# aliftffd/ViT-vs-Raw-IQ

Measured on AMD Instinct MI355X. Metric: IQ frames/sec training (fwd+loss+bwd+clip+AdamW), higher is better.
Workload: dtype bf16; 1 GPU; ViT-Tiny/16 224x224 C=1 19cls (BASELINE configs[1]); config_id=B, per_gpu_batch=256, global_batch=256, parallelism=dp1, hipgraph=True

## Files before the change

include/iqvit.h:

```cpp
#ifndef IQVIT_H
#define IQVIT_H
#include <stddef.h>
#include <stdint.h>

#ifdef __cplusplus
extern "C" {
#endif

typedef void* iq_stream_t;

enum { IQ_STATUS_OK = 0, IQ_STATUS_ARG = 1, IQ_STATUS_UNSUPPORTED = 2, IQ_STATUS_LAUNCH = 3 };

typedef struct iq_dropout {
  uint64_t seed;
  uint32_t step;
  uint32_t site;
  float p;
  const uint32_t* step_dev;
} iq_dropout_t;
#define IQ_SITE_IMPAIR 0xFFFFFFFFu
#define IQ_SITE_SYNTH 0xFFFFFFFEu

int iq_ln_supported(int D);
int iq_ln_fwd(const void* z, const float* gamma, const float* beta, void* x, float* mean, float* rstd, int M, int D,
              float eps, iq_stream_t stream);
size_t iq_ln_bwd_ws_bytes(int D);
int iq_ln_bwd(const void* dx, const void* z, const float* mean, const float* rstd, const float* gamma, void* dz,
              void* dy, const iq_dropout_t* drop, float* dgamma, float* dbeta, float* ws, int accumulate, int M,
              int D, iq_stream_t stream);
int iq_ln_bwd_partial_rows(int M, int D);

typedef struct iq_epilogue {
  const float* bias;
  int relu;
  const float* pe;
  int tok, seq, cls_off;
  iq_dropout_t drop;
  const void* gate;
  int ldg;
  float gate_scale;
  const void* residual;
  int ldr;
} iq_epilogue_t;
int iq_gemm_bf16_nt(const void* A, int lda, const void* B, int ldb, void* C, int ldc, int M, int N, int K,
                    const iq_epilogue_t* epi, iq_stream_t stream);
// ... 48 lines not shown
  const float* partials;
  int rows;
  int64_t row_stride;
  float* out;
  int64_t n;
} iq_reduce_seg_t;
size_t iq_wgrad_grouped_ws_bytes(const iq_wgrad_problem_t* probs, int nprob, int M, int max_workgroups);
int iq_gemm_bf16_wgrad_grouped(const iq_wgrad_problem_t* probs, int nprob, int M, float* ws, size_t ws_bytes,
                               int accumulate, int max_workgroups, const iq_reduce_seg_t* extra, int nextra,
                               iq_stream_t stream);

int iq_attn_supported(int S, int dh);
int iq_attn_fwd(const void* qkv, void* out, float* lse, int B, int S, int H, int dh, iq_stream_t stream);
int iq_attn_bwd(const void* qkv, const void* out, const void* dout, const float* lse, void* dqkv, int B, int S, int H,
                int dh, iq_stream_t stream);
int iq_attn_fwd_masked(const void* qkv, void* out, float* lse, const uint8_t* mask, long mask_hstride, int B, int S,
                       int H, int dh, iq_stream_t stream);
int iq_attn_bwd_masked(const void* qkv, const void* out, const void* dout, const float* lse, void* dqkv,
                       const uint8_t* mask, long mask_hstride, int B, int S, int H, int dh, iq_stream_t stream);
int iq_attn_probs(const void* qkv, const float* lse, float* out, long out_bstride, int B, int S, int H, int dh,
                  int rows, int heads, iq_stream_t stream);
int iq_attn_grad_probs(const void* qkv, const float* lse, const void* dout, float* out, long out_bstride, int B, int S,
                       int H, int dh, int rows, int heads, int positive, iq_stream_t stream);
int iq_attn_relevance_step(const void* qkv, const float* lse, const void* dout, const float* r_in, float* r_out, int B,
                           int S, int H, int dh, iq_stream_t stream);

int iq_frames_preprocess(const float* raw, float* out, int n_frames, int len, int take, const float* stats,
                         iq_stream_t stream);
typedef struct iq_impair {
  float phase_lo, phase_hi;
// ... 103 lines not shown
```

vit-vs-raw-iq_amd/_native.py:

```python
from __future__ import annotations

import ctypes as C
import os

_HERE = os.path.dirname(os.path.abspath(__file__))
LIB_PATH = os.environ.get("IQ_LIBIQVIT") or os.path.join(_HERE, "libiqvit.so")

BWD_PARAM_GRADS = 1

STATUS = {0: "ok", 1: "invalid argument", 2: "unsupported shape/configuration", 3: "HIP launch error"}


class IqError(RuntimeError):
    pass


class Dropout(C.Structure):
    _fields_ = [("seed", C.c_uint64), ("step", C.c_uint32), ("site", C.c_uint32), ("p", C.c_float),
                ("step_dev", C.c_void_p)]


class Impair(C.Structure):
    _fields_ = [("phase_lo", C.c_float), ("phase_hi", C.c_float), ("cfo_lo", C.c_float), ("cfo_hi", C.c_float),
                ("rot90", C.c_int), ("conj", C.c_int), ("shift_max", C.c_int), ("gain_db_lo", C.c_float),
# ... 31 lines not shown
    _fields_ = [("kind", C.c_int), ("in_channels", C.c_int), ("img_h", C.c_int), ("img_w", C.c_int),
                ("patch", C.c_int), ("seq_length", C.c_int), ("conv_k", C.c_int), ("use_cls", C.c_int),
                ("num_classes", C.c_int), ("d_model", C.c_int), ("n_head", C.c_int), ("n_layers", C.c_int),
                ("ffn_hidden", C.c_int), ("drop_prob", C.c_float)]


_P, _I, _Z, _F = C.c_void_p, C.c_int, C.c_size_t, C.c_float
_U64, _U32 = C.c_uint64, C.c_uint32

SIGNATURES = {
    "iq_ln_supported": (_I, [_I]),
    "iq_ln_fwd": (_I, [_P, _P, _P, _P, _P, _P, _I, _I, _F, _P]),
    "iq_ln_bwd_ws_bytes": (_Z, [_I]),
    "iq_ln_bwd_partial_rows": (_I, [_I, _I]),
    "iq_ln_bwd": (_I, [_P, _P, _P, _P, _P, _P, _P, C.POINTER(Dropout), _P, _P, _P, _I, _I, _I, _P]),
    "iq_gemm_bf16_nt": (_I, [_P, _I, _P, _I, _P, _I, _I, _I, _I, C.POINTER(Epilogue), _P]),
    "iq_gemm_ln_supported": (_I, [_I, _I]),
    "iq_gemm_bf16_ln": (_I, [_P, _I, _P, _I, _P, _P, _I, C.POINTER(Dropout), _P, _P, _F, _P, _P, _P, _P, _I, _I, _I, _P]),
    "iq_gemm_lnbwd_supported": (_I, [_I, _I]),
    "iq_gemm_lnbwd_partial_rows": (_I, [_I]),
    "iq_gemm_bf16_lnbwd": (_I, [_P, _I, _P, _I, _P, _I, _P, _P, _P, _P, C.POINTER(Dropout), _P, _P, _P, _I, _I, _I, _P]),
    "iq_ffn_chain_supported": (_I, [_I, _I, _I]),
    "iq_ffn_chain_bwd_partial_rows": (_I, [_I]),
    "iq_ffn_chain_bwd": (_I, [_P, _P, _P, _F, _P, _P, _P, _P, _P, _P, _P, C.POINTER(Dropout), _P, _P, _P, _P, _P, _I, _I, _I, _I, _P]),
    "iq_qkv_dgrad_ffn_chain_bwd": (_I, [_P, _P, _P, _P, _P, _P, _P, C.POINTER(Dropout), _P, _P, _P,
                                        _P, _P, _F, _P, _P, _P, _P, _P, _P, _P, C.POINTER(Dropout), _P, _P, _P, _P, _P, _I, _I, _I, _I, _P]),
    "iq_ffn_chain_gate_bytes": (_Z, [_I, _I]),
    "iq_ffn_chain_fwd": (_I, [_P, _P, _P, C.POINTER(Dropout), _P, _P, _P, C.POINTER(Dropout), _P, _P, _F, _P, _P, _P, _P, _P, _I, _I,
                              _I, _I, _P]),
    "iq_attn_out_ffn_chain_fwd": (_I, [_P, _P, _P, C.POINTER(Dropout), _P, _P, _P, _P, _P, _P, _P,
                                       _P, _P, C.POINTER(Dropout), _P, _P, _P, C.POINTER(Dropout), _P, _P, _F, _P, _P, _P, _P, _P,
                                       _P, _P, _P, _I, _I, _I, _I, _P]),
    "iq_wgrad_ws_bytes": (_Z, [_I, _I, _I]),
    "iq_gemm_bf16_wgrad": (_I, [_P, _I, _P, _I, _P, _P, _I, _I, _I, _P, _Z, _I, _P]),
    "iq_wgrad_grouped_ws_bytes": (_Z, [_P, _I, _I, _I]),
    "iq_gemm_bf16_wgrad_grouped": (_I, [_P, _I, _I, _P, _Z, _I, _I, _P, _I, _P]),
    "iq_attn_supported": (_I, [_I, _I]),
    "iq_attn_fwd": (_I, [_P, _P, _P, _I, _I, _I, _I, _P]),
    "iq_attn_bwd": (_I, [_P, _P, _P, _P, _P, _I, _I, _I, _I, _P]),
    "iq_attn_fwd_masked": (_I, [_P, _P, _P, _P, C.c_long, _I, _I, _I, _I, _P]),
    "iq_attn_bwd_masked": (_I, [_P, _P, _P, _P, _P, _P, C.c_long, _I, _I, _I, _I, _P]),
    "iq_attn_probs": (_I, [_P, _P, _P, C.c_long, _I, _I, _I, _I, _I, _I, _P]),
    "iq_attn_grad_probs": (_I, [_P, _P, _P, _P, C.c_long, _I, _I, _I, _I, _I, _I, _I, _P]),
    "iq_attn_relevance_step": (_I, [_P, _P, _P, _P, _P, _I, _I, _I, _I, _P]),
    "iq_frames_preprocess": (_I, [_P, _P, _I, _I, _I, C.POINTER(C.c_float), _P]),
    "iq_frames_impair": (_I, [_P, _P, _P, _I, _I, _I, C.POINTER(C.c_float), C.POINTER(Impair), _P]),
    "iq_frames_synth": (_I, [_P, _P, _P, _P, _P, _I, _I, C.POINTER(Synth), _P]),
    "iq_patchify": (_I, [_P, _P, _I, _I, _I, _I, _I, _I, _I, _P]),
    "iq_cls_rows": (_I, [_P, _P, _P, _I, _I, _I, C.POINTER(Dropout), _P]),
    "iq_embed_bwd_gather": (_I, [_P, _P, _P, _I, _I, _I, _I, _I, C.POINTER(Dropout), _I, _P]),
    "iq_embed_dgrad": (_I, [_P, _P, _I, _P, _I, _I, _I, _I, _I, _I, _I, _P]),
    "iq_linf_step": (_I, [_P, _P, _P, _F, _F, _F, _F, _Z, _P]),
    "iq_head_fwd": (_I, [_P, _P, _P, _P, _P, _P, _P, _P, _I, _I, _I, _I, _I, _P]),
    "iq_ce_fwd_bwd": (_I, [_P, _P, _I, _I, _F, _F, _P, _P, _P, _P]),
# ... 70 lines not shown
```

vit-vs-raw-iq_amd/csrc/attention.hip:

```cpp

#include "common.h"
#include "iqvit.h"
#include "prof.h"

namespace {

constexpr int ATT_THREADS = 512;
constexpr int ATT_WAVES = ATT_THREADS / 64;
constexpr float LOG2E = 1.4426950408889634f;
constexpr float LN2 = 0.6931471805599453f;
constexpr float NEG_BIG = -1.0e30f;

__device__ __forceinline__ float fast_exp2(float x) { return __builtin_amdgcn_exp2f(x); }

template <int DH> struct AttCfg {
  static constexpr int LD = (DH == 16) ? 16 : DH + 16;
  static constexpr int KS = (DH + 31) / 32;
  static constexpr int DT = DH / 16;
  static constexpr int CPR = DH / 8;
};

typedef __attribute__((address_space(3))) s16x4 lds_s16x4;

__device__ __forceinline__ bf16x8 tr_frag(const bf16* tile, int ld, int r0, int c0, int lane) {
// ... 467 lines not shown
      for (int i = 0; i < NIMG; ++i) v[i][j] = *reinterpret_cast<const bf16x8*>(base[i] + (long)r * ldg[i] + c * 8);
    }
#pragma unroll
    for (int j = 0; j < UN; ++j) {
      const int id = b0 + j * NT + tid;
      const int r = id >> 3, c = id & 7;
      if (id < total) {
        const bool live = r < S;
#pragma unroll
        for (int i = 0; i < NIMG; ++i) *reinterpret_cast<bf16x8*>(img[i] + once_off(r, c * 8)) = live ? v[i][j] : bf16x8{};
      }
    }
  }
}

template <int NT>
__global__ __launch_bounds__(NT, 4) void attn_bwd_once_kernel(const bf16* __restrict__ qkv, const bf16* __restrict__ out,
                                                              const bf16* __restrict__ dout, const float* __restrict__ lse,
                                                              bf16* __restrict__ dqkv, int S, int H, int spad, float scale) {
  constexpr int DH = 64, KS = 2, DT = 4, NW = NT / 64;
  extern __shared__ __attribute__((aligned(16))) unsigned char smem[];
  bf16* I0 = reinterpret_cast<bf16*>(smem);
  bf16* I1 = I0 + spad * ONCE_LD;
  float* lse_s = reinterpret_cast<float*>(I1 + spad * ONCE_LD);
  float* del_s = lse_s + spad;
  bf16* dSi = reinterpret_cast<bf16*>(del_s + spad);
  const int tid = threadIdx.x, lane = tid & 63, wave = tid >> 6, g = lane >> 4, c16 = lane & 15;
  const int b = blockIdx.x / H, h = blockIdx.x % H;
  const int D = H * DH;
  const long ldg = 3L * D;
  const bf16* qb = qkv + (long)b * S * ldg + h * DH;
  const bf16* kb_ = qb + D;
  const bf16* vb_ = qb + 2 * D;
  const bf16* ob = out + (long)b * S * D + h * DH;
  const bf16* dob = dout + (long)b * S * D + h * DH;
  bf16* dqb = dqkv + (long)b * S * ldg + h * DH;
  const float scale_log2 = scale * LOG2E;
  const int nunit = (S + 15) / 16;
  const int ldS = nunit * 16 + 8;

  {
    bf16* const img[2] = {I0, I1};
    const bf16* const src[2] = {qb, dob};
    const long lds_[2] = {ldg, (long)D};
    once_stage<NT, 2048 / NT, 2>(img, src, lds_, spad, S, tid);
  }
  __syncthreads();
  for (int q = tid; q < spad; q += NT) {
    float dl = 0.f, ls = 0.f;
    if (q < S) {
#pragma unroll
      for (int c = 0; c < 8; ++c) {
        const bf16x8 a = *reinterpret_cast<const bf16x8*>(I1 + once_off(q, c * 8));
        const bf16x8 o8 = *reinterpret_cast<const bf16x8*>(ob + (long)q * D + c * 8);
#pragma unroll
        for (int e = 0; e < 8; ++e) dl += (float)a[e] * (float)o8[e];
      }
      ls = lse[((long)b * H + h) * S + q] * LOG2E;
    }
    del_s[q] = dl;
    lse_s[q] = ls;
  }
  __syncthreads();

  for (int unit = wave; unit < nunit; unit += NW) {
    bf16x8 kf[KS], vf[KS];
#pragma unroll
    for (int s = 0; s < KS; ++s) {
      kf[s] = row_frag_gmem<DH>(kb_, ldg, unit * 16 + c16, S, s, lane);
      vf[s] = row_frag_gmem<DH>(vb_, ldg, unit * 16 + c16, S, s, lane);
    }
    f32x4 dv[DT], dk[DT];
#pragma unroll
    for (int dt = 0; dt < DT; ++dt) { dv[dt] = f32x4{0.f, 0.f, 0.f, 0.f}; dk[dt] = f32x4{0.f, 0.f, 0.f, 0.f}; }
    const int key = unit * 16 + c16;
    const bool unit_partial = unit * 16 + 16 > S;
    for (int ql = 0; ql < spad; ql += 32) {
      const bool u1 = ql + 16 < S;
      f32x4 p[2], ds[2];
#pragma unroll
      for (int u = 0; u < 2; ++u) {
        if (u == 1 && !u1) { p[1] = f32x4{0.f, 0.f, 0.f, 0.f}; ds[1] = f32x4{0.f, 0.f, 0.f, 0.f}; continue; }
        f32x4 sa = {0.f, 0.f, 0.f, 0.f}, dp = {0.f, 0.f, 0.f, 0.f};
#pragma unroll
        for (int s = 0; s < KS; ++s) {
          const bf16x8 qa = once_row_frag(I0, ql + u * 16 + c16, s, lane);
          const bf16x8 da = once_row_frag(I1, ql + u * 16 + c16, s, lane);
          sa = __builtin_amdgcn_mfma_f32_16x16x32_bf16(qa, kf[s], sa, 0, 0, 0);
          dp = __builtin_amdgcn_mfma_f32_16x16x32_bf16(da, vf[s], dp, 0, 0, 0);
        }
        const f32x4 lq4 = *reinterpret_cast<const f32x4*>(lse_s + ql + u * 16 + 4 * g);
        const f32x4 dl4 = *reinterpret_cast<const f32x4*>(del_s + ql + u * 16 + 4 * g);
// ... 31 lines not shown
        *reinterpret_cast<bf16x4*>(dqb + (long)key * ldg + 2 * D + dt * 16 + 4 * g) = wv;
      }
    }
  }

  __syncthreads();
  {
    bf16* const img[1] = {I0};
    const bf16* const src[1] = {kb_};
    const long lds_[1] = {ldg};
    once_stage<NT, 2048 / NT, 1>(img, src, lds_, spad, S, tid);
  }
  __syncthreads();
  for (int half = wave; half < nunit; half += NW) {
    const int q = half * 16 + c16;
    const bf16* drow = dSi + q * ldS + 4 * g;
    f32x4 dq[DT];
#pragma unroll
    for (int dt = 0; dt < DT; ++dt) dq[dt] = f32x4{0.f, 0.f, 0.f, 0.f};
    for (int kl = 0; kl < spad; kl += 32) {
      const bool k1 = kl + 16 < S;
      const bf16x4 lo = *reinterpret_cast<const bf16x4*>(drow + kl);
      bf16x4 hi = {};
      if (k1) hi = *reinterpret_cast<const bf16x4*>(drow + kl + 16);
      const bf16x8 dsB = {lo[0], lo[1], lo[2], lo[3], hi[0], hi[1], hi[2], hi[3]};
#pragma unroll
      for (int dt = 0; dt < DT; ++dt) {
        const bf16x8 kT = once_tr_frag(I0, kl, dt, lane);
        dq[dt] = __builtin_amdgcn_mfma_f32_16x16x32_bf16(kT, dsB, dq[dt], 0, 0, 0);
      }
    }
    if (q < S) {
#pragma unroll
      for (int dt = 0; dt < DT; ++dt) {
        bf16x4 w;
#pragma unroll
        for (int r = 0; r < 4; ++r) w[r] = (bf16)dq[dt][r];
        *reinterpret_cast<bf16x4*>(dqb + (long)q * ldg + dt * 16 + 4 * g) = w;
      }
    }
  }
}

template <int DH>
__device__ __forceinline__ bf16x8 row_frag_img(const bf16* tile, int ld, int row, int s, int lane) {
  const int d0 = s * 32 + 8 * (lane >> 4);
  bf16x8 v = {};
  if (DH >= 32 || d0 < DH) v = *reinterpret_cast<const bf16x8*>(tile + row * ld + d0);
  return v;
}

template <int UN>
__device__ __forceinline__ void stage_block(bf16* img, int ld, const bf16* src, int cols, int S, int spad, int tid, int nthr) {
  const int cpr = cols >> 3, total = spad * cpr, live = S * cpr;
  for (int base = 0; base < total; base += UN * nthr) {
    bf16x8 v[UN];
// ... 410 lines not shown
               long mask_hstride, int B, int S, int H, hipStream_t st) {
  const int spad = (S + 31) / 32 * 32;
  const int chunk = bwd_chunk_rows<DH>(S);
  if (S > ATT_MAX_S || chunk < 32) return IQ_ERR_UNSUPPORTED;
  const size_t lds = bwd_lds_bytes<DH>(S);
  if (lds > 48 * 1024)
    (void)hipFuncSetAttribute((const void*)attn_bwd_kernel<DH, MASKED>, hipFuncAttributeMaxDynamicSharedMemorySize, (int)lds);
  attn_bwd_kernel<DH, MASKED><<<B * H, ATT_THREADS, lds, st>>>((const bf16*)qkv, (const bf16*)out, (const bf16*)dout, lse,
                                                               (bf16*)dqkv, mask, mask_hstride, S, H, spad, chunk,
                                                               1.0f / sqrtf((float)DH), -10000.0f * sqrtf((float)DH));
  return iq_launch_status();
}

constexpr int ONCE_THREADS = 1024;
inline bool use_once(int S, int dh, bool masked) { return !masked && dh == 64 && (S + 31) / 32 * 32 <= ONCE_MAX_SPAD; }
template <int NT>
int launch_bwd_once(const void* qkv, const void* out, const void* dout, const float* lse, void* dqkv, int B, int S, int H,
                    hipStream_t st) {
  const int spad = (S + 31) / 32 * 32, nunit = (S + 15) / 16;
  const size_t lds = (size_t)2 * spad * ONCE_LD * 2 + (size_t)2 * spad * sizeof(float) + (size_t)spad * (nunit * 16 + 8) * 2;
  auto k = attn_bwd_once_kernel<NT>;
  if (lds > 48 * 1024) (void)hipFuncSetAttribute((const void*)k, hipFuncAttributeMaxDynamicSharedMemorySize, (int)lds);
  k<<<B * H, NT, lds, st>>>((const bf16*)qkv, (const bf16*)out, (const bf16*)dout, lse, (bf16*)dqkv, S, H, spad,
                            1.0f / sqrtf(64.0f));
  return iq_launch_status();
}

template <bool MASKED>
int dispatch_fwd(const void* qkv, void* out, float* lse, const uint8_t* mask, long hs, int B, int S, int H, int dh,
                 hipStream_t st) {
  switch (dh) {
    case 16: return launch_fwd<16, MASKED>(qkv, out, lse, mask, hs, B, S, H, st);
    case 32: return launch_fwd<32, MASKED>(qkv, out, lse, mask, hs, B, S, H, st);
    case 64: return launch_fwd<64, MASKED>(qkv, out, lse, mask, hs, B, S, H, st);
    default: return IQ_ERR_UNSUPPORTED;
  }
}
template <bool MASKED>
int dispatch_bwd(const void* qkv, const void* out, const void* dout, const float* lse, void* dqkv, const uint8_t* mask,
                 long hs, int B, int S, int H, int dh, hipStream_t st) {
  switch (dh) {
    case 16: return launch_bwd<16, MASKED>(qkv, out, dout, lse, dqkv, mask, hs, B, S, H, st);
    case 32: return launch_bwd<32, MASKED>(qkv, out, dout, lse, dqkv, mask, hs, B, S, H, st);
    case 64: return launch_bwd<64, MASKED>(qkv, out, dout, lse, dqkv, mask, hs, B, S, H, st);
    default: return IQ_ERR_UNSUPPORTED;
  }
}

}

extern "C" int iq_attn_supported(int S, int dh) {
  if (S <= 0 || S > ATT_MAX_S) return 0;
  return (dh == 16 || dh == 32 || dh == 64) ? 1 : 0;
}

extern "C" int iq_attn_fwd_masked(const void* qkv, void* out, float* lse, const uint8_t* mask, long mask_hstride, int B,
                                  int S, int H, int dh, iq_stream_t stream) {
  if (B <= 0) return IQ_OK;
  if (!qkv || !out || !lse || S <= 0 || H <= 0) return IQ_ERR_ARG;
  if (mask_hstride != 0 && mask_hstride != (long)S * S) return IQ_ERR_ARG;
  hipStream_t st = (hipStream_t)stream;
// ... 37 lines not shown
  if (frame) {
    switch (dh) {
      case 16: return launch_frame_bwd<16>(qkv, out, dout, lse, dqkv, B, S, H, st);
      case 32: return launch_frame_bwd<32>(qkv, out, dout, lse, dqkv, B, S, H, st);
      default: return launch_frame_bwd<64>(qkv, out, dout, lse, dqkv, B, S, H, st);
    }
  }
  if (once) return launch_bwd_once<ONCE_THREADS>(qkv, out, dout, lse, dqkv, B, S, H, st);
  return mask ? dispatch_bwd<true>(qkv, out, dout, lse, dqkv, mask, mask_hstride, B, S, H, dh, st)
              : dispatch_bwd<false>(qkv, out, dout, lse, dqkv, nullptr, 0, B, S, H, dh, st);
}
extern "C" int iq_attn_bwd(const void* qkv, const void* out, const void* dout, const float* lse, void* dqkv, int B,
                           int S, int H, int dh, iq_stream_t stream) {
  return iq_attn_bwd_masked(qkv, out, dout, lse, dqkv, nullptr, 0, B, S, H, dh, stream);
}
```

vit-vs-raw-iq_amd/csrc/layernorm.hip:

```cpp
#include "common.h"
#include "iqvit.h"
#include "prof.h"

namespace {

template <int LPR>
__device__ __forceinline__ float group_sum(float v) {
#pragma unroll
  for (int o = LPR / 2; o > 0; o >>= 1) v += __shfl_xor(v, o, 64);
  return v;
}

constexpr int LN_THREADS = 256;

template <int LPR, int NV, bool MASK = false>
__global__ __launch_bounds__(LN_THREADS) void ln_fwd_kernel(const bf16* __restrict__ Z, const float* __restrict__ gamma,
                                                            const float* __restrict__ beta, bf16* __restrict__ X,
                                                            float* __restrict__ mean_out, float* __restrict__ rstd_out,
                                                            int M, int D, float eps) {
  constexpr int RPW = 64 / LPR;
  constexpr int RPB = RPW * (LN_THREADS / 64);
  const int lane = threadIdx.x & 63, wave = threadIdx.x >> 6;
  const int j = lane % LPR, rsub = lane / LPR;
  float g[NV][8], b[NV][8];
// ... 32 lines not shown
        float y[8];
#pragma unroll
        for (int e = 0; e < 8; ++e) y[e] = g[v][e] * ((x[v][e] - mean) * rstd) + b[v][e];
        if (!MASK || (v * LPR + j) * 8 < D) *reinterpret_cast<bf16x8*>(X + row * D + (v * LPR + j) * 8) = pack8(y);
      }
      if (j == 0) { mean_out[row] = mean; rstd_out[row] = rstd; }
    }
  }
}

template <int LPR, int NV, bool DROP, bool MASK = false>
__global__ __launch_bounds__(LN_THREADS) void ln_bwd_kernel(const bf16* __restrict__ dX, const bf16* __restrict__ Z,
                                                            const float* __restrict__ mean_in, const float* __restrict__ rstd_in,
                                                            const float* __restrict__ gamma, bf16* __restrict__ dZ,
                                                            bf16* __restrict__ dY, IqRng rng, uint32_t thresh, float dscale,
                                                            float* __restrict__ partial, int M, int D) {
  constexpr int RPW = 64 / LPR;
  constexpr int RPB = RPW * (LN_THREADS / 64);
  extern __shared__ __attribute__((aligned(16))) float red[];
  const int lane = threadIdx.x & 63, wave = threadIdx.x >> 6;
  const int j = lane % LPR, rsub = lane / LPR;
  float g[NV][8], ag[NV][8], ab[NV][8];
#pragma unroll
  for (int v = 0; v < NV; ++v) {
    const int c = (v * LPR + j) * 8;
#pragma unroll
    for (int e = 0; e < 8; ++e) { g[v][e] = (!MASK || c < D) ? gamma[c + e] : 0.f; ag[v][e] = 0.f; ab[v][e] = 0.f; }
  }
  const float invD = 1.0f / (float)D;
  if (DROP) rng = rng_resolve(rng);
  for (long row0 = (long)blockIdx.x * RPB; row0 < M; row0 += (long)gridDim.x * RPB) {
    const long row = row0 + wave * RPW + rsub;
    const bool ok = row < M;
    float xh[NV][8], dy[NV][8];
    float mean = 0.f, rstd = 0.f;
    if (ok) { mean = mean_in[row]; rstd = rstd_in[row]; }
    float s1 = 0.f, s2 = 0.f;
#pragma unroll
    for (int v = 0; v < NV; ++v) {
      bf16x8 tz = {}, td = {};
      const bool cv = !MASK || (v * LPR + j) * 8 < D;
      if (ok && cv) {
        tz = *reinterpret_cast<const bf16x8*>(Z + row * D + (v * LPR + j) * 8);
        td = *reinterpret_cast<const bf16x8*>(dX + row * D + (v * LPR + j) * 8);
      }
      unpack8(tz, xh[v]);
      unpack8(td, dy[v]);
#pragma unroll
      for (int e = 0; e < 8; ++e) {
        xh[v][e] = cv ? (xh[v][e] - mean) * rstd : 0.f;
        ag[v][e] += dy[v][e] * xh[v][e];
        ab[v][e] += dy[v][e];
        dy[v][e] *= g[v][e];
        s1 += dy[v][e];
        s2 += dy[v][e] * xh[v][e];
      }
    }
    const float c1 = group_sum<LPR>(s1) * invD;
    const float c2 = group_sum<LPR>(s2) * invD;
    if (ok) {
#pragma unroll
      for (int v = 0; v < NV; ++v) {
        float o[8];
#pragma unroll
        for (int e = 0; e < 8; ++e) o[e] = rstd * (dy[v][e] - c1 - xh[v][e] * c2);
        const long off = row * D + (v * LPR + j) * 8;
        if (MASK && (v * LPR + j) * 8 >= D) continue;
        *reinterpret_cast<bf16x8*>(dZ + off) = pack8(o);
        if (DROP) {
          const uint32_t keep = dropout_keep8(rng, (uint64_t)off >> 3, thresh);
#pragma unroll
          for (int e = 0; e < 8; ++e) o[e] = ((keep >> e) & 1u) ? o[e] * dscale : 0.f;
          *reinterpret_cast<bf16x8*>(dY + off) = pack8(o);
        }
      }
    }
  }
  const int rslot = wave * RPW + rsub;
#pragma unroll
  for (int v = 0; v < NV; ++v) {
    const int c = (v * LPR + j) * 8;
// ... 110 lines not shown

extern "C" size_t iq_ln_bwd_ws_bytes(int D) { return (size_t)LN_MAX_BLOCKS * 2 * D * sizeof(float); }

extern "C" int iq_ln_bwd_partial_rows(int M, int D) {
  LnShape s;
  if (M <= 0 || !ln_shape(D, &s)) return 0;
  int rows = 0;
  bool ok = ln_dispatch(s, [&](auto lpr, auto nv) {
    constexpr int LPR = decltype(lpr)::value;
    rows = ln_grid(M, (64 / LPR) * 4);
  });
  if (!ok) rows = ln_grid(M, 4);
  return rows;
}

extern "C" int iq_ln_bwd(const void* dx, const void* z, const float* mean, const float* rstd, const float* gamma,
                         void* dz, void* dy, const iq_dropout_t* drop, float* dgamma, float* dbeta, float* ws,
                         int accumulate, int M, int D, iq_stream_t stream) {
  LnShape s;
  if (M <= 0) return IQ_OK;
  if (!dx || !z || !mean || !rstd || !gamma || !dz || !ws) return IQ_ERR_ARG;
  if ((dgamma == nullptr) != (dbeta == nullptr)) return IQ_ERR_ARG;
  const bool reduce_now = dgamma != nullptr;
  if (!ln_shape(D, &s)) return IQ_ERR_UNSUPPORTED;
  int dropping; IqRng rng; uint32_t thresh; float dscale;
  (void)dropout_unpack(drop, &dropping, &rng, &thresh, &dscale);
  if (dropping && !dy) return IQ_ERR_ARG;
  hipStream_t st = (hipStream_t)stream;
  IQ_PROF(IQ_FAM_LN_BWD, st);
  IQ_PROF_K(2.0 * (double)M * D * (3 + (dropping ? 1 : 0)) + 8.0 * M, 0.0, "ln_bwd_kernel(D=%d)", D);
  int rc = IQ_OK;
  bool ok = ln_dispatch(s, [&](auto lpr, auto nv) {
    constexpr int LPR = decltype(lpr)::value, NV = decltype(nv)::value;
    constexpr int RPB = (64 / LPR) * 4;
    const int nblk = ln_grid(M, RPB);
    const size_t lds = (size_t)RPB * 2 * D * sizeof(float);
    if (lds > 160 * 1024) { rc = IQ_ERR_UNSUPPORTED; return; }
    if (dropping) {
      auto k = ln_bwd_kernel<LPR, NV, true>;
      if (lds > 48 * 1024) (void)hipFuncSetAttribute((const void*)k, hipFuncAttributeMaxDynamicSharedMemorySize, (int)lds);
      k<<<nblk, LN_THREADS, lds, st>>>((const bf16*)dx, (const bf16*)z, mean, rstd, gamma, (bf16*)dz, (bf16*)dy, rng,
                                       thresh, dscale, ws, M, D);
    } else {
      auto k = ln_bwd_kernel<LPR, NV, false>;
      if (lds > 48 * 1024) (void)hipFuncSetAttribute((const void*)k, hipFuncAttributeMaxDynamicSharedMemorySize, (int)lds);
      k<<<nblk, LN_THREADS, lds, st>>>((const bf16*)dx, (const bf16*)z, mean, rstd, gamma, (bf16*)dz, (bf16*)dy, rng,
                                       thresh, dscale, ws, M, D);
    }
    if (reduce_now) ln_bwd_reduce_kernel<<<(2 * D + 31) / 32, 1024, 0, st>>>(ws, nblk, D, dgamma, dbeta, accumulate);
  });
  if (!ok) ok = ln_dispatch_masked(D, [&](auto nv) {
    constexpr int NV = decltype(nv)::value;
    constexpr int RPB = 4;
    const int nblk = ln_grid(M, RPB);
    const size_t lds = (size_t)RPB * 2 * D * sizeof(float);
    if (dropping)
      ln_bwd_kernel<64, NV, true, true><<<nblk, LN_THREADS, lds, st>>>((const bf16*)dx, (const bf16*)z, mean, rstd, gamma,
                                                                      (bf16*)dz, (bf16*)dy, rng, thresh, dscale, ws, M, D);
    else
      ln_bwd_kernel<64, NV, false, true><<<nblk, LN_THREADS, lds, st>>>((const bf16*)dx, (const bf16*)z, mean, rstd, gamma,
                                                                       (bf16*)dz, (bf16*)dy, rng, thresh, dscale, ws, M, D);
    if (reduce_now) ln_bwd_reduce_kernel<<<(2 * D + 31) / 32, 1024, 0, st>>>(ws, nblk, D, dgamma, dbeta, accumulate);
  });
  if (!ok) return IQ_ERR_UNSUPPORTED;
  return rc != IQ_OK ? rc : iq_launch_status();
}
```

vit-vs-raw-iq_amd/csrc/model.hip:

```cpp
#include <hip/hip_runtime.h>
#include <stdio.h>
#include <string.h>

#include <string>
#include <vector>

#include "attn_maps.h"
#include "common.h"
#include "iqvit.h"
#include "prof.h"

int head_bwd_dx_launch(const float* dlogits, const float* featn, const float* hstat, const float* ln_g, const float* W, void* dx,
                       int B, int S, int D, int K, int pool, hipStream_t st);
int embed_bwd_gather_launch(const void* dx0, void* demb, int B, int S, int tok, int D, int has_cls, const iq_dropout_t* drop,
                            hipStream_t st);

namespace {

struct Entry {
  std::string name;
  size_t off;
  int ndim;
  int dims[4];
};
// ... 110 lines not shown
  std::vector<LayerOff> L;
  size_t hln_g, hln_b, head_w, head_b, head_begin;
  size_t sh_flat, sh_embw, sh_table, shadow_bytes;
  std::vector<TransDesc> ttab;
  int ttiles = 0;
  const void* table_uploaded_to = nullptr;
  float* params = nullptr;
  float* grads = nullptr;
  const float* pe = nullptr;
  unsigned char* shadow = nullptr;
  std::string err;
  uint32_t* step_ctr = nullptr;
  uint64_t last_seed = 0;
  bool last_tr = false;
  bool last_train_fwd = false;
  const void* fwd_ws = nullptr;
  int fwd_batch = 0;

  iq_dropout_t bwd_site(uint32_t id, const uint32_t* step_dev, bool tr) const {
    iq_dropout_t d;
    d.seed = last_seed; d.step = 0; d.site = id; d.p = tr ? c.drop_prob : 0.f; d.step_dev = step_dev;
    return d;
  }

  size_t add(const std::string& name, std::vector<int> dims, size_t& cur, bool aligned = true) {
    if (aligned) cur = align_up(cur, 64);
    Entry e;
    e.name = name; e.off = cur; e.ndim = (int)dims.size();
    size_t n = 1;
    for (int i = 0; i < 4; ++i) { e.dims[i] = i < e.ndim ? dims[i] : 1; n *= (size_t)e.dims[i]; }
// ... 446 lines not shown
  const WsPlan w = plan_ws(m, batch);
  if (ws_bytes < w.total) return fail(m, IQ_ERR_ARG, "backward: workspace too small");
  hipStream_t st = (hipStream_t)stream;
  unsigned char* ws = (unsigned char*)workspace;
  const int D = c.d_model, F = c.ffn_hidden, S = m->S, H = c.n_head, B = batch, K = c.num_classes;
  const int M = B * S, MT = B * m->tok;
  const bool tr = m->last_tr;
  const uint32_t* step_dev = m->step_ctr ? m->step_ctr : (const uint32_t*)(ws + w.step_ctr);
  const float* P = m->params;
  float* G = m->grads;
  float* wws = (float*)(ws + w.wgrad_ws);
  const float dscale = tr ? dropout_scale(c.drop_prob) : 1.f;

  if (stage_hi == Lr + 1) {
    if (!dlogits && !denc) return fail(m, IQ_ERR_ARG, "backward: dlogits or denc required at the head stage");
    if (dlogits && !pgrads) {
      IQ_TRY(head_bwd_dx_launch(dlogits, (const float*)(ws + w.head_feat), (const float*)(ws + w.head_stat),
                                m->head_ln ? P + m->hln_g : nullptr, P + m->head_w, ws + w.gA, B, S, D, K, m->pool, st), "head bwd (dx)");
    } else if (dlogits) {
      IQ_TRY(iq_head_bwd(dlogits, (const float*)(ws + w.head_feat), (const float*)(ws + w.head_stat),
                         m->head_ln ? P + m->hln_g : nullptr, m->head_ln ? P + m->hln_b : nullptr, P + m->head_w,
                         G + m->head_w, G + m->head_b, m->head_ln ? G + m->hln_g : nullptr,
                         m->head_ln ? G + m->hln_b : nullptr, ws + w.gA, B, S, D, K, m->pool, accumulate, stream), "head bwd");
    } else if (!accumulate && pgrads) {
      (void)hipMemsetAsync(G + m->head_begin, 0, (m->nparam - m->head_begin) * sizeof(float), st);
    }
    if (denc) f32_into_bf16_kernel<<<blocks_for((size_t)M * D / 8), 256, 0, st>>>(denc, (bf16*)(ws + w.gA), (size_t)M * D / 8, dlogits ? 1 : 0);
  }
  const bool fuse1 = iq_gemm_lnbwd_supported(D, F) != 0, fuse2 = iq_gemm_lnbwd_supported(D, 3 * D) != 0;
  const Route route = layer_route(M, S, D, F);
  const bool chain = fuse1 && m->last_train_fwd && route.chain;
  bool deferred = false;
  for (int sidx = (stage_hi > Lr ? Lr : stage_hi); sidx >= 1 && sidx >= stage_lo; --sidx) {
    const int l = sidx - 1;
    const LayerOff& o = m->L[l];
    const WsPlan::L& a = w.layers[l];
    const unsigned char* xin = l == 0 ? ws + w.x0 : ws + w.layers[l - 1].x2;
    unsigned char *gZ = ws + w.gZ, *gY = ws + w.gY, *gZ1 = ws + w.gZ1, *gY1 = ws + w.gY1;
    unsigned char *gH = ws + w.gH, *gQKV = ws + w.gQKV;
    iq_epilogue_t e;
    float* lp2 = (float*)(ws + w.ln_part[0]);
    float* lp1 = (float*)(ws + w.ln_part[1]);
    const bool norm2_here = l == Lr - 1 || !fuse2;
    if (norm2_here) {
      const iq_dropout_t dr2 = m->bwd_site(3 + 3 * l, step_dev, tr);
      IQ_TRY(iq_ln_bwd(ws + w.gA, ws + a.z2, (const float*)(ws + a.mean2), (const float*)(ws + a.rstd2), P + o.g2,
                       gZ, gY, &dr2, nullptr, nullptr, lp2, accumulate, M, D, stream), "norm2 bwd");
    }
    const unsigned char* dO2 = tr ? gY : gZ;
    const unsigned char* dAo = tr ? gY1 : gZ1;
    const iq_wgrad_problem_t wg[4] = {
        {dO2, D, ws + a.hid, F, G + o.w2, G + o.b2, D, F},
        {gH, F, ws + a.x1, D, G + o.w1, G + o.b1, F, D},
        {dAo, D, ws + a.att, D, G + o.wo, G + o.bo, D, D},
        {gQKV, 3 * D, xin, D, G + o.wqkv, G + o.bqkv, 3 * D, D}};
    const int rows2 = norm2_here ? iq_ln_bwd_partial_rows(M, D) : deferred ? iq_ffn_chain_bwd_partial_rows(M) : iq_gemm_lnbwd_partial_rows(M);
    const int rows1 = chain ? iq_ffn_chain_bwd_partial_rows(M) : fuse1 ? iq_gemm_lnbwd_partial_rows(M) : iq_ln_bwd_partial_rows(M, D);
    const iq_reduce_seg_t lnseg[4] = {{lp2, rows2, 2L * D, G + o.g2, D}, {lp2 + D, rows2, 2L * D, G + o.be2, D},
                                      {lp1, rows1, 2L * D, G + o.g1, D}, {lp1 + D, rows1, 2L * D, G + o.be1, D}};
// ... 26 lines not shown
      }
    }
    if (!chain) IQ_TRY(iq_gemm_bf16_nt(dAo, D, m->sht(o.t_wo), D, ws + w.gAtt, D, M, D, D, nullptr, stream), "out-proj dgrad");
    if (rh) {
      const float* lse = (const float*)(ws + a.lse);
      if (rh->maps && rh->maps[l])
        IQ_TRY(iq_attn_grad_probs(ws + a.qkv, lse, ws + w.gAtt, rh->maps[l], rh->bstride, B, S, H, m->dh, rh->rows, rh->heads,
                                  rh->positive, stream), "gradient-weighted attention map");
      if (rh->rel) {
        const int i = Lr - 1 - l;
        IQ_TRY(attn_relevance_step_launch(ws + a.qkv, lse, ws + w.gAtt, i ? rh->r[(i - 1) & 1] : nullptr, l ? rh->r[i & 1] : rh->rel,
                                          B, S, H, m->dh, i ? 0 : m->has_cls ? 1 : 2, st), "relevance step");
      }
      if (l == 0) break;
    }
    IQ_TRY(iq_attn_bwd(ws + a.qkv, ws + a.att, ws + w.gAtt, (const float*)(ws + a.lse), gQKV, B, S, H, m->dh, stream), "attention bwd");
    if (pgrads) IQ_TRY(iq_gemm_bf16_wgrad_grouped(wg, 4, M, wws, w.wgrad_ws_bytes, accumulate, 0, lnseg, 4, stream), "layer weight gradients");
    deferred = l > 0 && fuse2 && chain && route.chain_takes_qkv_dgrad && sidx - 1 >= stage_lo;
    if (deferred) continue;
    if (l > 0 && fuse2) {
      const LayerOff& ob = m->L[l - 1];
      const WsPlan::L& ab = w.layers[l - 1];
      const iq_dropout_t dr2b = m->bwd_site(3 + 3 * (l - 1), step_dev, tr);
      IQ_TRY(iq_gemm_bf16_lnbwd(gQKV, 3 * D, m->sht(o.t_wqkv), 3 * D, gZ1, D, ws + ab.z2, (const float*)(ws + ab.mean2),
                                (const float*)(ws + ab.rstd2), P + ob.g2, &dr2b, gZ, gY, lp2, M, D, 3 * D, stream),
             "qkv dgrad + norm2 bwd of the layer below");
    } else {
      memset(&e, 0, sizeof(e));
      e.residual = gZ1; e.ldr = D;
      IQ_TRY(iq_gemm_bf16_nt(gQKV, 3 * D, m->sht(o.t_wqkv), 3 * D, ws + w.gA, D, M, D, 3 * D, &e, stream), "qkv dgrad");
    }
// ... 82 lines not shown
```

Baseline: 52990 frames/s.

## Exploit CLS-only head gradient to sparsify top-layer norm2 and attention backward

When the classifier uses only the CLS token, the head backward now emits gradients for that single row, and the top layer's norm2 backward runs only on CLS rows after zeroing the other rows. Attention backward for the top layer gets a CLS-query variant that processes just the first query tile and writes zeros for the remaining dQ rows. The aim is to skip work in the last layer whose upstream gradient is zero for all non-CLS tokens. In exchange it adds memsets, new kernels and a strided row mapping in the layernorm backward. The FFN and weight-gradient GEMMs still run over the full M rows.

```diff
diff --git a/include/iqvit.h b/include/iqvit.h
--- a/include/iqvit.h
+++ b/include/iqvit.h
@@ -29,6 +29,9 @@
               void* dy, const iq_dropout_t* drop, float* dgamma, float* dbeta, float* ws, int accumulate, int M,
               int D, iq_stream_t stream);
 int iq_ln_bwd_partial_rows(int M, int D);
+int iq_ln_bwd_rows(const void* dx, const void* z, const float* mean, const float* rstd, const float* gamma, void* dz,
+                   void* dy, const iq_dropout_t* drop, float* dgamma, float* dbeta, float* ws, int accumulate, int M,
+                   int D, int rs, iq_stream_t stream);
 
 typedef struct iq_epilogue {
   const float* bias;
@@ -107,6 +110,9 @@
 int iq_attn_fwd(const void* qkv, void* out, float* lse, int B, int S, int H, int dh, iq_stream_t stream);
 int iq_attn_bwd(const void* qkv, const void* out, const void* dout, const float* lse, void* dqkv, int B, int S, int H,
                 int dh, iq_stream_t stream);
+int iq_attn_bwd_cls(const void* qkv, const void* out, const void* dout, const float* lse, void* dqkv, int B, int S, int H,
+                    int dh, iq_stream_t stream);
+int iq_attn_bwd_cls_same_bits(int S, int H, int dh);
 int iq_attn_fwd_masked(const void* qkv, void* out, float* lse, const uint8_t* mask, long mask_hstride, int B, int S,
                        int H, int dh, iq_stream_t stream);
 int iq_attn_bwd_masked(const void* qkv, const void* out, const void* dout, const float* lse, void* dqkv,
diff --git a/vit-vs-raw-iq_amd/_native.py b/vit-vs-raw-iq_amd/_native.py
--- a/vit-vs-raw-iq_amd/_native.py
+++ b/vit-vs-raw-iq_amd/_native.py
@@ -69,6 +69,7 @@
     "iq_ln_bwd_ws_bytes": (_Z, [_I]),
     "iq_ln_bwd_partial_rows": (_I, [_I, _I]),
     "iq_ln_bwd": (_I, [_P, _P, _P, _P, _P, _P, _P, C.POINTER(Dropout), _P, _P, _P, _I, _I, _I, _P]),
+    "iq_ln_bwd_rows": (_I, [_P, _P, _P, _P, _P, _P, _P, C.POINTER(Dropout), _P, _P, _P, _I, _I, _I, _I, _P]),
     "iq_gemm_bf16_nt": (_I, [_P, _I, _P, _I, _P, _I, _I, _I, _I, C.POINTER(Epilogue), _P]),
     "iq_gemm_ln_supported": (_I, [_I, _I]),
     "iq_gemm_bf16_ln": (_I, [_P, _I, _P, _I, _P, _P, _I, C.POINTER(Dropout), _P, _P, _F, _P, _P, _P, _P, _I, _I, _I, _P]),
@@ -93,6 +94,8 @@
     "iq_attn_supported": (_I, [_I, _I]),
     "iq_attn_fwd": (_I, [_P, _P, _P, _I, _I, _I, _I, _P]),
     "iq_attn_bwd": (_I, [_P, _P, _P, _P, _P, _I, _I, _I, _I, _P]),
+    "iq_attn_bwd_cls": (_I, [_P, _P, _P, _P, _P, _I, _I, _I, _I, _P]),
+    "iq_attn_bwd_cls_same_bits": (_I, [_I, _I, _I]),
     "iq_attn_fwd_masked": (_I, [_P, _P, _P, _P, C.c_long, _I, _I, _I, _I, _P]),
     "iq_attn_bwd_masked": (_I, [_P, _P, _P, _P, _P, _P, C.c_long, _I, _I, _I, _I, _P]),
     "iq_attn_probs": (_I, [_P, _P, _P, C.c_long, _I, _I, _I, _I, _I, _I, _P]),
diff --git a/vit-vs-raw-iq_amd/csrc/attention.hip b/vit-vs-raw-iq_amd/csrc/attention.hip
--- a/vit-vs-raw-iq_amd/csrc/attention.hip
+++ b/vit-vs-raw-iq_amd/csrc/attention.hip
@@ -505,11 +505,12 @@
   }
 }
 
-template <int NT>
-__global__ __launch_bounds__(NT, 4) void attn_bwd_once_kernel(const bf16* __restrict__ qkv, const bf16* __restrict__ out,
-                                                              const bf16* __restrict__ dout, const float* __restrict__ lse,
-                                                              bf16* __restrict__ dqkv, int S, int H, int spad, float scale) {
+template <int NT, bool CLS>
+__device__ __forceinline__ void once_body(const bf16* __restrict__ qkv, const bf16* __restrict__ out,
+                                          const bf16* __restrict__ dout, const float* __restrict__ lse,
+                                          bf16* __restrict__ dqkv, int S, int H, int spad, float scale) {
   constexpr int DH = 64, KS = 2, DT = 4, NW = NT / 64;
+  const int qrows = CLS ? 32 : spad;
   extern __shared__ __attribute__((aligned(16))) unsigned char smem[];
   bf16* I0 = reinterpret_cast<bf16*>(smem);
   bf16* I1 = I0 + spad * ONCE_LD;
@@ -534,10 +535,10 @@
     bf16* const img[2] = {I0, I1};
     const bf16* const src[2] = {qb, dob};
     const long lds_[2] = {ldg, (long)D};
-    once_stage<NT, 2048 / NT, 2>(img, src, lds_, spad, S, tid);
+    once_stage<NT, 2048 / NT, 2>(img, src, lds_, qrows, S, tid);
   }
   __syncthreads();
-  for (int q = tid; q < spad; q += NT) {
+  for (int q = tid; q < qrows; q += NT) {
     float dl = 0.f, ls = 0.f;
     if (q < S) {
 #pragma unroll
@@ -566,7 +567,7 @@
     for (int dt = 0; dt < DT; ++dt) { dv[dt] = f32x4{0.f, 0.f, 0.f, 0.f}; dk[dt] = f32x4{0.f, 0.f, 0.f, 0.f}; }
     const int key = unit * 16 + c16;
     const bool unit_partial = unit * 16 + 16 > S;
-    for (int ql = 0; ql < spad; ql += 32) {
+    for (int ql = 0; ql < qrows; ql += 32) {
       const bool u1 = ql + 16 < S;
       f32x4 p[2], ds[2];
 #pragma unroll
@@ -628,6 +629,13 @@
   __syncthreads();
   for (int half = wave; half < nunit; half += NW) {
     const int q = half * 16 + c16;
+    if (CLS && half > 0) {
+      if (q < S) {
+#pragma unroll
+        for (int dt = 0; dt < DT; ++dt) *reinterpret_cast<bf16x4*>(dqb + (long)q * ldg + dt * 16 + 4 * g) = bf16x4{};
+      }
+      continue;
+    }
     const bf16* drow = dSi + q * ldS + 4 * g;
     f32x4 dq[DT];
 #pragma unroll
@@ -654,6 +662,19 @@
       }
     }
   }
+}
+
+template <int NT>
+__global__ __launch_bounds__(NT, 4) void attn_bwd_once_kernel(const bf16* __restrict__ qkv, const bf16* __restrict__ out,
+                                                              const bf16* __restrict__ dout, const float* __restrict__ lse,
+                                                              bf16* __restrict__ dqkv, int S, int H, int spad, float scale) {
+  once_body<NT, false>(qkv, out, dout, lse, dqkv, S, H, spad, scale);
+}
+template <int NT>
+__global__ __launch_bounds__(NT, 4) void attn_bwd_cls_once_kernel(const bf16* __restrict__ qkv, const bf16* __restrict__ out,
+                                                                  const bf16* __restrict__ dout, const float* __restrict__ lse,
+                                                                  bf16* __restrict__ dqkv, int S, int H, int spad, float scale) {
+  once_body<NT, true>(qkv, out, dout, lse, dqkv, S, H, spad, scale);
 }
 
 template <int DH>
@@ -1094,12 +1115,12 @@
 
 constexpr int ONCE_THREADS = 1024;
 inline bool use_once(int S, int dh, bool masked) { return !masked && dh == 64 && (S + 31) / 32 * 32 <= ONCE_MAX_SPAD; }
-template <int NT>
+template <int NT, bool CLS = false>
 int launch_bwd_once(const void* qkv, const void* out, const void* dout, const float* lse, void* dqkv, int B, int S, int H,
                     hipStream_t st) {
   const int spad = (S + 31) / 32 * 32, nunit = (S + 15) / 16;
   const size_t lds = (size_t)2 * spad * ONCE_LD * 2 + (size_t)2 * spad * sizeof(float) + (size_t)spad * (nunit * 16 + 8) * 2;
-  auto k = attn_bwd_once_kernel<NT>;
+  auto k = CLS ? attn_bwd_cls_once_kernel<NT> : attn_bwd_once_kernel<NT>;
   if (lds > 48 * 1024) (void)hipFuncSetAttribute((const void*)k, hipFuncAttributeMaxDynamicSharedMemorySize, (int)lds);
   k<<<B * H, NT, lds, st>>>((const bf16*)qkv, (const bf16*)out, (const bf16*)dout, lse, (bf16*)dqkv, S, H, spad,
                             1.0f / sqrtf(64.0f));
@@ -1125,6 +1146,87 @@
     case 64: return launch_bwd<64, MASKED>(qkv, out, dout, lse, dqkv, mask, hs, B, S, H, st);
     default: return IQ_ERR_UNSUPPORTED;
   }
+}
+
+constexpr int CLS_THREADS = 256;
+template <int W>
+__device__ __forceinline__ float lanes_sum(float v) {
+#pragma unroll
+  for (int o = W / 2; o > 0; o >>= 1) v += __shfl_xor(v, o, 64);
+  return v;
+}
+template <int DH>
+__global__ __launch_bounds__(CLS_THREADS) void attn_bwd_cls_kernel(const bf16* __restrict__ qkv, const bf16* __restrict__ out,
+                                                                   const bf16* __restrict__ dout, const float* __restrict__ lse,
+                                                                   bf16* __restrict__ dqkv, int S, int H, float scale) {
+  constexpr int CPR = AttCfg<DH>::CPR, G = CLS_THREADS / CPR;
+  __shared__ float red[G * DH];
+  const int tid = threadIdx.x, c = tid % CPR, grp = tid / CPR;
+  const int b = blockIdx.x / H, h = blockIdx.x % H;
+  const int D = H * DH;
+  const long ldg = 3L * D;
+  const bf16* qb = qkv + (long)b * S * ldg + h * DH + c * 8;
+  const bf16* kb_ = qb + D;
+  const bf16* vb_ = qb + 2 * D;
+  bf16* dqb = dqkv + (long)b * S * ldg + h * DH + c * 8;
+  float q[8], dO[8];
+  unpack8(*reinterpret_cast<const bf16x8*>(qb), q);
+  unpack8(*reinterpret_cast<const bf16x8*>(dout + (long)b * S * D + h * DH + c * 8), dO);
+  float delta = 0.f;
+#pragma unroll
+  for (int cc = 0; cc < CPR; ++cc) {
+    const bf16x8 a = *reinterpret_cast<const bf16x8*>(dout + (long)b * S * D + h * DH + cc * 8);
+    const bf16x8 o8 = *reinterpret_cast<const bf16x8*>(out + (long)b * S * D + h * DH + cc * 8);
+#pragma unroll
+    for (int e = 0; e < 8; ++e) delta += (float)a[e] * (float)o8[e];
+  }
+  const float ls = lse[((long)b * H + h) * S] * LOG2E;
+  const float scale_log2 = scale * LOG2E;
+  float acc[8];
+#pragma unroll
+  for (int e = 0; e < 8; ++e) acc[e] = 0.f;
+  for (int k0 = 0; k0 < S; k0 += G) {
+    const int key = k0 + grp;
+    const bool live = key < S;
+    const long row = (long)(live ? key : S - 1) * ldg;
+    float kf[8], vf[8];
+    unpack8(*reinterpret_cast<const bf16x8*>(kb_ + row), kf);
+    unpack8(*reinterpret_cast<const bf16x8*>(vb_ + row), vf);
+    float s = 0.f, dp = 0.f;
+#pragma unroll
+    for (int e = 0; e < 8; ++e) { s += q[e] * kf[e]; dp += dO[e] * vf[e]; }
+    s = lanes_sum<CPR>(s);
+    dp = lanes_sum<CPR>(dp);
+    const float pv = fast_exp2(s * scale_log2 - ls);
+    const float p = (float)(bf16)pv;
+    const float ds = (float)(bf16)(pv * (dp - delta) * scale);
+    if (live) {
+      float dv[8], dk[8];
+#pragma unroll
+      for (int e = 0; e < 8; ++e) { dv[e] = p * dO[e]; dk[e] = ds * q[e]; acc[e] += ds * kf[e]; }
+      *reinterpret_cast<bf16x8*>(dqb + row + D) = pack8(dk);
+      *reinterpret_cast<bf16x8*>(dqb + row + 2 * D) = pack8(dv);
+      if (key > 0) *reinterpret_cast<bf16x8*>(dqb + row) = bf16x8{};
+    }
+  }
+#pragma unroll
+  for (int e = 0; e < 8; ++e) red[grp * DH + c * 8 + e] = acc[e];
+  __syncthreads();
+  if (tid < DH) {
+    float t = 0.f;
+    for (int g2 = 0; g2 < G; ++g2) t += red[g2 * DH + tid];
+    red[tid] = t;
+  }
+  __syncthreads();
+  if (tid < CPR) *reinterpret_cast<bf16x8*>(dqb) = pack8(red + tid * 8);
+}
+
+template <int DH>
+int launch_bwd_cls(const void* qkv, const void* out, const void* dout, const float* lse, void* dqkv, int B, int S, int H,
+                   hipStream_t st) {
+  attn_bwd_cls_kernel<DH><<<B * H, CLS_THREADS, 0, st>>>((const bf16*)qkv, (const bf16*)out, (const bf16*)dout, lse, (bf16*)dqkv,
+                                                         S, H, 1.0f / sqrtf((float)DH));
+  return iq_launch_status();
 }
 
 }
@@ -1192,3 +1294,27 @@
                            int S, int H, int dh, iq_stream_t stream) {
   return iq_attn_bwd_masked(qkv, out, dout, lse, dqkv, nullptr, 0, B, S, H, dh, stream);
 }
+
+extern "C" int iq_attn_bwd_cls(const void* qkv, const void* out, const void* dout, const float* lse, void* dqkv, int B,
+                               int S, int H, int dh, iq_stream_t stream) {
+  if (B <= 0) return IQ_OK;
+  if (!qkv || !out || !dout || !lse || !dqkv || S <= 0 || H <= 0) return IQ_ERR_ARG;
+  if (S > ATT_MAX_S) return IQ_ERR_UNSUPPORTED;
+  hipStream_t st = (hipStream_t)stream;
+  IQ_PROF(IQ_FAM_ATTN_BWD, st);
+  if (use_once(S, dh, false) && !use_frame(S, frame_bwd_lds(S, H, dh))) {
+    IQ_PROF_K(2.0 * B * S * 5.0 * H * dh + 4.0 * B * H, 10.0 * B * H * (double)S * dh, "attn_bwd_cls_once_kernel<%d>", ONCE_THREADS);
+    return launch_bwd_once<ONCE_THREADS, true>(qkv, out, dout, lse, dqkv, B, S, H, st);
+  }
+  IQ_PROF_K(2.0 * B * S * 5.0 * H * dh + 4.0 * B * H, 10.0 * B * H * (double)S * dh, "attn_bwd_cls_kernel<%d>", dh);
+  switch (dh) {
+    case 16: return launch_bwd_cls<16>(qkv, out, dout, lse, dqkv, B, S, H, st);
+    case 32: return launch_bwd_cls<32>(qkv, out, dout, lse, dqkv, B, S, H, st);
+    case 64: return launch_bwd_cls<64>(qkv, out, dout, lse, dqkv, B, S, H, st);
+    default: return IQ_ERR_UNSUPPORTED;
+  }
+}
+
+extern "C" int iq_attn_bwd_cls_same_bits(int S, int H, int dh) {
+  return (use_once(S, dh, false) && !use_frame(S, frame_bwd_lds(S, H, dh))) ? 1 : 0;
+}
diff --git a/vit-vs-raw-iq_amd/csrc/layernorm.hip b/vit-vs-raw-iq_amd/csrc/layernorm.hip
--- a/vit-vs-raw-iq_amd/csrc/layernorm.hip
+++ b/vit-vs-raw-iq_amd/csrc/layernorm.hip
@@ -70,7 +70,7 @@
                                                             const float* __restrict__ mean_in, const float* __restrict__ rstd_in,
                                                             const float* __restrict__ gamma, bf16* __restrict__ dZ,
                                                             bf16* __restrict__ dY, IqRng rng, uint32_t thresh, float dscale,
-                                                            float* __restrict__ partial, int M, int D) {
+                                                            float* __restrict__ partial, int M, int D, long rs) {
   constexpr int RPW = 64 / LPR;
   constexpr int RPB = RPW * (LN_THREADS / 64);
   extern __shared__ __attribute__((aligned(16))) float red[];
@@ -87,18 +87,19 @@
   if (DROP) rng = rng_resolve(rng);
   for (long row0 = (long)blockIdx.x * RPB; row0 < M; row0 += (long)gridDim.x * RPB) {
     const long row = row0 + wave * RPW + rsub;
-    const bool ok = row < M;
+    const bool ok = row < M && (rs == 1 || row % rs == 0);
+    const long frow = row;
     float xh[NV][8], dy[NV][8];
     float mean = 0.f, rstd = 0.f;
-    if (ok) { mean = mean_in[row]; rstd = rstd_in[row]; }
+    if (ok) { mean = mean_in[frow]; rstd = rstd_in[frow]; }
     float s1 = 0.f, s2 = 0.f;
 #pragma unroll
     for (int v = 0; v < NV; ++v) {
       bf16x8 tz = {}, td = {};
       const bool cv = !MASK || (v * LPR + j) * 8 < D;
       if (ok && cv) {
-        tz = *reinterpret_cast<const bf16x8*>(Z + row * D + (v * LPR + j) * 8);
-        td = *reinterpret_cast<const bf16x8*>(dX + row * D + (v * LPR + j) * 8);
+        tz = *reinterpret_cast<const bf16x8*>(Z + frow * D + (v * LPR + j) * 8);
+        td = *reinterpret_cast<const bf16x8*>(dX + (row / rs) * D + (v * LPR + j) * 8);
       }
       unpack8(tz, xh[v]);
       unpack8(td, dy[v]);
@@ -120,7 +121,7 @@
         float o[8];
 #pragma unroll
         for (int e = 0; e < 8; ++e) o[e] = rstd * (dy[v][e] - c1 - xh[v][e] * c2);
-        const long off = row * D + (v * LPR + j) * 8;
+        const long off = frow * D + (v * LPR + j) * 8;
         if (MASK && (v * LPR + j) * 8 >= D) continue;
         *reinterpret_cast<bf16x8*>(dZ + off) = pack8(o);
         if (DROP) {
@@ -261,11 +262,13 @@
   return rows;
 }
 
-extern "C" int iq_ln_bwd(const void* dx, const void* z, const float* mean, const float* rstd, const float* gamma,
-                         void* dz, void* dy, const iq_dropout_t* drop, float* dgamma, float* dbeta, float* ws,
-                         int accumulate, int M, int D, iq_stream_t stream) {
+extern "C" int iq_ln_bwd_rows(const void* dx, const void* z, const float* mean, const float* rstd, const float* gamma,
+                              void* dz, void* dy, const iq_dropout_t* drop, float* dgamma, float* dbeta, float* ws,
+                              int accumulate, int M, int D, int rs, iq_stream_t stream) {
   LnShape s;
   if (M <= 0) return IQ_OK;
+  if (rs < 1 || (long)M * rs > 0x7fffffffL) return IQ_ERR_ARG;
+  M *= rs;
   if (!dx || !z || !mean || !rstd || !gamma || !dz || !ws) return IQ_ERR_ARG;
   if ((dgamma == nullptr) != (dbeta == nullptr)) return IQ_ERR_ARG;
   const bool reduce_now = dgamma != nullptr;
@@ -287,12 +290,12 @@
       auto k = ln_bwd_kernel<LPR, NV, true>;
       if (lds > 48 * 1024) (void)hipFuncSetAttribute((const void*)k, hipFuncAttributeMaxDynamicSharedMemorySize, (int)lds);
       k<<<nblk, LN_THREADS, lds, st>>>((const bf16*)dx, (const bf16*)z, mean, rstd, gamma, (bf16*)dz, (bf16*)dy, rng,
-                                       thresh, dscale, ws, M, D);
+                                       thresh, dscale, ws, M, D, (long)rs);
     } else {
       auto k = ln_bwd_kernel<LPR, NV, false>;
       if (lds > 48 * 1024) (void)hipFuncSetAttribute((const void*)k, hipFuncAttributeMaxDynamicSharedMemorySize, (int)lds);
       k<<<nblk, LN_THREADS, lds, st>>>((const bf16*)dx, (const bf16*)z, mean, rstd, gamma, (bf16*)dz, (bf16*)dy, rng,
-                                       thresh, dscale, ws, M, D);
+                                       thresh, dscale, ws, M, D, (long)rs);
     }
     if (reduce_now) ln_bwd_reduce_kernel<<<(2 * D + 31) / 32, 1024, 0, st>>>(ws, nblk, D, dgamma, dbeta, accumulate);
   });
@@ -303,12 +306,18 @@
     const size_t lds = (size_t)RPB * 2 * D * sizeof(float);
     if (dropping)
       ln_bwd_kernel<64, NV, true, true><<<nblk, LN_THREADS, lds, st>>>((const bf16*)dx, (const bf16*)z, mean, rstd, gamma,
-                                                                      (bf16*)dz, (bf16*)dy, rng, thresh, dscale, ws, M, D);
+                                                                      (bf16*)dz, (bf16*)dy, rng, thresh, dscale, ws, M, D, (long)rs);
     else
       ln_bwd_kernel<64, NV, false, true><<<nblk, LN_THREADS, lds, st>>>((const bf16*)dx, (const bf16*)z, mean, rstd, gamma,
-                                                                       (bf16*)dz, (bf16*)dy, rng, thresh, dscale, ws, M, D);
+                                                                       (bf16*)dz, (bf16*)dy, rng, thresh, dscale, ws, M, D, (long)rs);
     if (reduce_now) ln_bwd_reduce_kernel<<<(2 * D + 31) / 32, 1024, 0, st>>>(ws, nblk, D, dgamma, dbeta, accumulate);
   });
   if (!ok) return IQ_ERR_UNSUPPORTED;
   return rc != IQ_OK ? rc : iq_launch_status();
 }
+
+extern "C" int iq_ln_bwd(const void* dx, const void* z, const float* mean, const float* rstd, const float* gamma,
+                         void* dz, void* dy, const iq_dropout_t* drop, float* dgamma, float* dbeta, float* ws,
+                         int accumulate, int M, int D, iq_stream_t stream) {
+  return iq_ln_bwd_rows(dx, z, mean, rstd, gamma, dz, dy, drop, dgamma, dbeta, ws, accumulate, M, D, 1, stream);
+}
diff --git a/vit-vs-raw-iq_amd/csrc/model.hip b/vit-vs-raw-iq_amd/csrc/model.hip
--- a/vit-vs-raw-iq_amd/csrc/model.hip
+++ b/vit-vs-raw-iq_amd/csrc/model.hip
@@ -148,6 +148,7 @@
   uint64_t last_seed = 0;
   bool last_tr = false;
   bool last_train_fwd = false;
+  bool last_cls_top = false;
   const void* fwd_ws = nullptr;
   int fwd_batch = 0;
 
@@ -624,14 +625,16 @@
 
   if (stage_hi == Lr + 1) {
     if (!dlogits && !denc) return fail(m, IQ_ERR_ARG, "backward: dlogits or denc required at the head stage");
+    m->last_cls_top = m->has_cls && m->pool == 0 && denc == nullptr && dlogits != nullptr && Lr > 0;
+    const int Sh = m->last_cls_top ? 1 : S;
     if (dlogits && !pgrads) {
       IQ_TRY(head_bwd_dx_launch(dlogits, (const float*)(ws + w.head_feat), (const float*)(ws + w.head_stat),
-                                m->head_ln ? P + m->hln_g : nullptr, P + m->head_w, ws + w.gA, B, S, D, K, m->pool, st), "head bwd (dx)");
+                                m->head_ln ? P + m->hln_g : nullptr, P + m->head_w, ws + w.gA, B, Sh, D, K, m->pool, st), "head bwd (dx)");
     } else if (dlogits) {
       IQ_TRY(iq_head_bwd(dlogits, (const float*)(ws + w.head_feat), (const float*)(ws + w.head_stat),
                          m->head_ln ? P + m->hln_g : nullptr, m->head_ln ? P + m->hln_b : nullptr, P + m->head_w,
                          G + m->head_w, G + m->head_b, m->head_ln ? G + m->hln_g : nullptr,
-                         m->head_ln ? G + m->hln_b : nullptr, ws + w.gA, B, S, D, K, m->pool, accumulate, stream), "head bwd");
+                         m->head_ln ? G + m->hln_b : nullptr, ws + w.gA, B, Sh, D, K, m->pool, accumulate, stream), "head bwd");
     } else if (!accumulate && pgrads) {
       (void)hipMemsetAsync(G + m->head_begin, 0, (m->nparam - m->head_begin) * sizeof(float), st);
     }
@@ -652,7 +655,14 @@
     float* lp2 = (float*)(ws + w.ln_part[0]);
     float* lp1 = (float*)(ws + w.ln_part[1]);
     const bool norm2_here = l == Lr - 1 || !fuse2;
-    if (norm2_here) {
+    const bool cls_top = sidx == Lr && m->last_cls_top;
+    if (cls_top) {
+      const iq_dropout_t dr2 = m->bwd_site(3 + 3 * l, step_dev, tr);
+      (void)hipMemsetAsync(gZ, 0, (size_t)M * D * 2, st);
+      if (tr) (void)hipMemsetAsync(gY, 0, (size_t)M * D * 2, st);
+      IQ_TRY(iq_ln_bwd_rows(ws + w.gA, ws + a.z2, (const float*)(ws + a.mean2), (const float*)(ws + a.rstd2), P + o.g2,
+                            gZ, gY, &dr2, nullptr, nullptr, lp2, accumulate, B, D, S, stream), "norm2 bwd (CLS rows)");
+    } else if (norm2_here) {
       const iq_dropout_t dr2 = m->bwd_site(3 + 3 * l, step_dev, tr);
       IQ_TRY(iq_ln_bwd(ws + w.gA, ws + a.z2, (const float*)(ws + a.mean2), (const float*)(ws + a.rstd2), P + o.g2,
                        gZ, gY, &dr2, nullptr, nullptr, lp2, accumulate, M, D, stream), "norm2 bwd");
@@ -709,7 +719,8 @@
       }
       if (l == 0) break;
     }
-    IQ_TRY(iq_attn_bwd(ws + a.qkv, ws + a.att, ws + w.gAtt, (const float*)(ws + a.lse), gQKV, B, S, H, m->dh, stream), "attention bwd");
+    if (cls_top && iq_attn_bwd_cls_same_bits(S, H, m->dh)) IQ_TRY(iq_attn_bwd_cls(ws + a.qkv, ws + a.att, ws + w.gAtt, (const float*)(ws + a.lse), gQKV, B, S, H, m->dh, stream), "attention bwd (CLS query)");
+    else IQ_TRY(iq_attn_bwd(ws + a.qkv, ws + a.att, ws + w.gAtt, (const float*)(ws + a.lse), gQKV, B, S, H, m->dh, stream), "attention bwd");
     if (pgrads) IQ_TRY(iq_gemm_bf16_wgrad_grouped(wg, 4, M, wws, w.wgrad_ws_bytes, accumulate, 0, lnseg, 4, stream), "layer weight gradients");
     deferred = l > 0 && fuse2 && chain && route.chain_takes_qkv_dgrad && sidx - 1 >= stage_lo;
     if (deferred) continue;
```

Result: no change. 53480 frames/s (median of 6 runs) (+0.9%).
